# apache/cassandra

Hardware: AMD Instinct MI355X
Metric: compaction MB/s (input SSTable bytes merged+compressed) (higher is better)
Workload: dtype u8; 1 GPU; C2: 8x2GiB sstables, 10% key overlap, ~1KiB values, LZ4 16KiB chunks; sstables=8, overlap_pct=10, clustering_rows=0, tombstone_pct=0, range_tomb_pct=0, parallelism=token-independent shards x1, no collectives, storage=/tmp/gpuc_bench, input_uncompressed_bytes_per_rank=17182763435

## Files before the change

### cassandra_amd/csrc/gpucompact.cpp

```cpp
#include "kernels.hip"
#include "kernels_rows.hip"
#include "bti_core.h"
#include "sstable_meta.h"
#include "sstable_out.h"
#include "../../include/gpucompact.h"

#include <algorithm>
#include <cmath>
#include <cstdio>
#include <cstring>
#include <map>
#include <set>
#include <memory>
#include <mutex>
#include <stdexcept>
#include <string>
#include <thread>
#include <future>
#include <functional>
#include <atomic>
#include <fcntl.h>
#include <unistd.h>
#include <vector>

// ... 666 lines not shown
    m.has_partition_deletions = hst.has_partition_deletions != 0;
    memcpy(m.part_size_hist, hst.part_size_hist, sizeof(m.part_size_hist));
    memcpy(m.cells_hist, hst.cells_hist, sizeof(m.cells_hist));
}

struct OutputImage {
    uint64_t g0 = 0, g1 = 0;
    uint64_t total_unc = 0, total_idx = 0;
    uint32_t n_chunks = 0;
    const DevBuf *slots = nullptr, *csize = nullptr, *ccrc = nullptr;
    const DevBuf *out_index = nullptr, *bloom = nullptr;
    uint8_t* h_index = nullptr;
    uint64_t words = 0;
    HBloomSpec bs{};
    OutStats hst{};
    const std::vector<Event>* ev_c = nullptr;
    bool index_late = false;
};

static void drain_and_finish(const OutputImage& im, const OutPartsBuf& opb, const SerParams2& sp,
                             const DevBuf& d_tomb, uint32_t tomb_cap, const TableTypes& types,
                             const OutputOptions& opt, hipStream_t stream, hipStream_t cstream,
                             hipEvent_t ev2, hipEvent_t ev4, WriteDeviceOut& w) {
    const std::string& out_base = opt.base;
    const bool snappy_out = opt.snappy, bti_out = opt.bti;
    const int wslot = opt.wslot;
    const uint32_t OCL = opt.chunk_len;
    const uint32_t SLOT_STRIDE = snappy_out ? snp_slot_stride(OCL) : lz4_slot_stride(OCL);
    const uint32_t SLAB = (512u << 20) / OCL;
    const uint32_t n_chunks = im.n_chunks;
    const uint32_t n_slabs = n_chunks ? (n_chunks + SLAB - 1) / SLAB : 0;
    const uint64_t total_unc = im.total_unc, total_idx = im.total_idx, words = im.words;
    uint8_t* const h_index = im.h_index;
    const OutStats& hst = im.hst;
    const HBloomSpec& bs = im.bs;
    std::string data_path = out_base + "-Data.db";
    write_file(data_path, nullptr, 0);
    const uint64_t worst_slab = (uint64_t)SLAB * ((uint64_t)SLOT_STRIDE + 4);
    const int NSLOTS = 4;
    uint8_t* h_slab0 = (uint8_t*)g_pin_out[wslot][0].get(worst_slab * NSLOTS);
    if (!h_slab0) throw std::runtime_error("pinned out alloc failed");
    DevBuf d_gat[2], d_foff[2];
    if (n_slabs) {
        d_gat[0].alloc(worst_slab); d_gat[1].alloc(worst_slab);
        d_foff[0].alloc((uint64_t)SLAB * 8); d_foff[1].alloc((uint64_t)SLAB * 8);
    }
    std::vector<uint32_t> cs(n_chunks);
    std::vector<uint64_t> foff_h[2];
    foff_h[0].resize(SLAB); foff_h[1].resize(SLAB);
    std::future<void> wfut[NSLOTS];
    double t_drain0 = 0, t_drain1 = 0;
    {
        struct timespec tsd; clock_gettime(CLOCK_MONOTONIC, &tsd);
        t_drain0 = tsd.tv_sec * 1e3 + tsd.tv_nsec / 1e6;
    }
    uint64_t file_off = 0;
    double tw_comp = 0, tw_d2h = 0, tw_wfut = 0;
    auto wallm = []() {
        struct timespec t; clock_gettime(CLOCK_MONOTONIC, &t);
        return t.tv_sec * 1e3 + t.tv_nsec / 1e6;
    };
    for (uint32_t i = 0; i < n_slabs; i++) {
        uint32_t cb = i * SLAB, m = std::min(SLAB, n_chunks - cb);
        HIP_CHECK(hipStreamWaitEvent(cstream, (*im.ev_c)[i], 0));
        HIP_CHECK(hipMemcpyAsync(cs.data() + cb, im.csize->as<uint32_t>() + cb, (uint64_t)m * 4,
                                 hipMemcpyDeviceToHost, cstream));
        double tq0 = wallm();
        HIP_CHECK(hipStreamSynchronize(cstream));
        tw_comp += wallm() - tq0;
        auto& fo = foff_h[i & 1];
        uint64_t acc = 0;
        for (uint32_t j = 0; j < m; j++) { fo[j] = acc; acc += cs[cb + j]; }
        uint64_t slab_bytes = acc + (uint64_t)m * 4;
        HIP_CHECK(hipMemcpyAsync(d_foff[i & 1].p, fo.data(), (uint64_t)m * 8,
                                 hipMemcpyHostToDevice, cstream));
        hipLaunchKernelGGL(k_chunk_gather, dim3(m), dim3(WAVE), 0, cstream,
                           im.slots->as<uint8_t>() + (uint64_t)cb * SLOT_STRIDE,
                           im.csize->as<uint32_t>() + cb, im.ccrc->as<uint32_t>() + cb,
                           d_foff[i & 1].as<uint64_t>(), d_gat[i & 1].as<uint8_t>(), m,
                           SLOT_STRIDE);
        int slot = (int)(i % NSLOTS);
        double tq1 = wallm();
        if (wfut[slot].valid()) wfut[slot].get();
        tw_wfut += wallm() - tq1;
        uint8_t* hbuf = h_slab0 + (uint64_t)slot * worst_slab;
        HIP_CHECK(hipMemcpyAsync(hbuf, d_gat[i & 1].p, slab_bytes, hipMemcpyDeviceToHost, cstream));
        double tq2 = wallm();
        HIP_CHECK(hipStreamSynchronize(cstream));
        tw_d2h += wallm() - tq2;
        uint64_t off0 = file_off;
        wfut[slot] = std::async(std::launch::async, [=]() {
            pwrite_range(data_path, hbuf, slab_bytes, off0, 4);
        });
        file_off += slab_bytes;
    }
    {
        double tq3 = wallm();
        for (int sfin = 0; sfin < NSLOTS; sfin++)
            if (wfut[sfin].valid()) wfut[sfin].get();
        tw_wfut += wallm() - tq3;
    }
    if (g_trace)
        fprintf(stderr, "[drain] slabs=%u wait_compress=%.0fms wait_d2h=%.0fms wait_write=%.0fms\n",
                n_slabs, tw_comp, tw_d2h, tw_wfut);
    {
        struct timespec tsd; clock_gettime(CLOCK_MONOTONIC, &tsd);
        t_drain1 = tsd.tv_sec * 1e3 + tsd.tv_nsec / 1e6;
    }
    w.compressed_len = file_off;
    TR("wsd: drain done");
    if (im.index_late) {
        HIP_CHECK(hipStreamWaitEvent(cstream, ev2, 0));
        HIP_CHECK(hipMemcpyAsync(h_index, im.out_index->p, total_idx, hipMemcpyDeviceToHost, cstream));
        HIP_CHECK(hipStreamSynchronize(cstream));
    }
    HIP_CHECK(hipEventRecord(ev4, stream));

    {
        std::vector<uint8_t> h_bloom(words * 8);
        std::vector<uint32_t> h_crc(n_chunks);
        TR("wsd: tail vectors");
        HIP_CHECK(hipMemcpy(h_bloom.data(), im.bloom->p, words * 8, hipMemcpyDeviceToHost));
        TR("wsd: bloom d2h");
        if (n_chunks)
            HIP_CHECK(hipMemcpy(h_crc.data(), im.ccrc->p, (uint64_t)n_chunks * 4, hipMemcpyDeviceToHost));
        HIP_CHECK(hipStreamSynchronize(stream));
        HIP_CHECK(hipStreamSynchronize(cstream));
        TR("wsd: tail synced");
        std::future<uint32_t> fut_digest =
            std::async(std::launch::async, [&]() { return fold_digest(h_crc, cs); });
        std::future<bytes> fut_summary;
        if (!bti_out)
            fut_summary = std::async(std::launch::async,
                                     [&]() { return summary_db(h_index, total_idx); });

        std::vector<uint32_t> tombs;
        if (hst.tomb_count) {
            uint64_t nt = std::min<uint64_t>(hst.tomb_count, tomb_cap);
            tombs.resize(nt);
            HIP_CHECK(hipMemcpy(tombs.data(), d_tomb.p, nt * 4, hipMemcpyDeviceToHost));
            if (hst.tomb_count > tomb_cap)
                throw std::runtime_error("tombstone list overflow (internal cap)");
        }
        OutMeta m{};
        {
            const uint64_t n_groups = im.g1 - im.g0;
            DevBuf d_kh;
            d_kh.alloc(n_groups * 8 + 8);
            uint32_t blocks = (uint32_t)((n_groups + 255) / 256);
            if (n_groups)
                hipLaunchKernelGGL(k_key_hash2, dim3(blocks), dim3(256), 0, stream, opb.op,
                                   im.g1, d_kh.as<uint64_t>(), im.g0);
            std::vector<uint64_t> kh(n_groups);
            std::vector<uint8_t> keep(n_groups);
            if (n_groups) {
                HIP_CHECK(hipStreamSynchronize(stream));
                HIP_CHECK(hipMemcpy(kh.data(), d_kh.p, n_groups * 8, hipMemcpyDeviceToHost));
                HIP_CHECK(hipMemcpy(keep.data(), opb.op.keep + im.g0, n_groups, hipMemcpyDeviceToHost));
            }
            m.key_hashes.reserve(n_groups);
            for (uint64_t g2 = 0; g2 < n_groups; g2++)
                if (keep[g2]) m.key_hashes.push_back(kh[g2]);
        }
        fill_meta_from_stats(m, hst, sp.hs, types);
        for (uint32_t tv : tombs) m.tomb_hist[tv]++;
        m.compression_ratio = total_unc ? (double)(w.compressed_len - (uint64_t)n_chunks * 4) / (double)total_unc : -1.0;
        if (hst.partitions_out) {
            uint64_t fg = hst.first_group, lg = hst.last_group;
            for (int which = 0; which < 2; which++) {
                uint64_t g = which ? lg : fg;
                uint64_t ka;
                uint16_t kl;
                HIP_CHECK(hipMemcpy(&ka, opb.op.key_addr + g, 8, hipMemcpyDeviceToHost));
                HIP_CHECK(hipMemcpy(&kl, opb.op.klen + g, 2, hipMemcpyDeviceToHost));
                bytes kb(kl);
                HIP_CHECK(hipMemcpy(kb.data(), (const void*)ka, kl, hipMemcpyDeviceToHost));
                (which ? m.last_key : m.first_key) = kb;
            }
        }
        TR("wsd: meta built");
        uint32_t digest = fut_digest.get();

        TR("wsd: digest done");
        struct timespec ts0, ts1;
        clock_gettime(CLOCK_MONOTONIC, &ts0);
        if (bti_out) {
            bti::bytes parts_img, rows_img;
            std::vector<int32_t> ckw;
            for (auto& t : types.clustering_types) ckw.push_back(type_width(t));
            build_bti_from_index_image(h_index, total_idx, total_unc, ckw, &parts_img, &rows_img);
            write_file(out_base + "-Partitions.db", parts_img);
            write_file(out_base + "-Rows.db", rows_img);
        } else {
            write_file_parallel(out_base + "-Index.db", h_index, total_idx, 4);
        }
        write_file(out_base + "-Filter.db", filter_db(bs.k, h_bloom));
        write_file(out_base + "-CompressionInfo.db",
                   compression_info_db(snappy_out, OCL, total_unc, cs));
        write_file(out_base + "-Digest.crc32", digest_text(digest));
        write_file(out_base + "-Statistics.db", serialize_statistics_out(m));
        if (!bti_out) write_file(out_base + "-Summary.db", fut_summary.get());
        write_file(out_base + "-TOC.txt", toc_text(bti_out));
        clock_gettime(CLOCK_MONOTONIC, &ts1);
        TR("wsd: components written");
        w.ms_io = (ts1.tv_sec - ts0.tv_sec) * 1e3 + (ts1.tv_nsec - ts0.tv_nsec) / 1e6;
        w.ms_d2h = t_drain1 - t_drain0;
    }
}

static WriteDeviceOut write_sstable_device(const OutPartsBuf& opb, const UnfColsBuf& rows,
                                           uint64_t n_groups, SerParams2 sp, DevBuf& d_stats,
                                           DevBuf& d_tomb, uint32_t tomb_cap,
                                           const TableTypes& types, const OutputOptions& opt,
                                           hipStream_t stream) {
    WriteDeviceOut w;
    if (!chunk_len_supported(opt.chunk_len))
        throw unsupported_error("unsupported output chunk_length " + std::to_string(opt.chunk_len) +
                                CHUNK_LEN_WHY);
    const std::string& out_base = opt.base;
    const bool snappy_out = opt.snappy, bti_out = opt.bti;
    const int wslot = opt.wslot;
    const uint32_t OCL = opt.chunk_len;
// ... 48 lines not shown
    w.rows = hst.rows_out;
    w.cells = hst.total_cells;

    HBloomSpec bs = bloom_spec_001();
    uint64_t num_bits = w.partitions * (uint64_t)bs.buckets + 20;
    uint64_t words = num_bits ? ((num_bits - 1) >> 6) + 1 : 1;
    DevBuf d_out_data, d_out_index, d_bloom;
    d_out_data.alloc(total_unc);
    d_out_index.alloc(total_idx);
    d_bloom.alloc(words * 8);
    HIP_CHECK(hipMemsetAsync(d_bloom.p, 0, words * 8, stream));
    HIP_CHECK(hipEventRecord(ev1, stream));
    int NSEG = n_groups >= 4096 && total_unc > (256ull << 20) ? 8 : 1;
    if (const char* e = getenv("GPUC_NSEG")) NSEG = std::max(1, std::min(64, atoi(e)));
    if (n_groups < 4096) NSEG = 1;
    std::vector<uint64_t> seg_g(NSEG + 1), seg_end_byte(NSEG);
    if (NSEG > 1) {
        seg_g[0] = 0;
        seg_g[NSEG] = n_groups;
        for (int j = 1; j < NSEG; j++) seg_g[j] = n_groups * (uint64_t)j / NSEG;
        for (int j = 0; j < NSEG - 1; j++)
            HIP_CHECK(hipMemcpy(&seg_end_byte[j], d_psize.as<uint64_t>() + seg_g[j + 1], 8,
                                hipMemcpyDeviceToHost));
        seg_end_byte[NSEG - 1] = total_unc;
    } else {
        seg_g[0] = 0;
        seg_g[NSEG] = n_groups;
        seg_end_byte[NSEG - 1] = total_unc;
    }
    auto launch_serialize_seg = [&](int j) {
        uint32_t waves_per_block = 4;
        uint64_t gs = seg_g[j], ge = seg_g[j + 1];
        uint64_t blocks = (std::max<uint64_t>(ge - gs, 1) + waves_per_block - 1) / waves_per_block;
        if (ge > gs)
            hipLaunchKernelGGL(k_serialize_rows, dim3((uint32_t)blocks),
                               dim3(WAVE * waves_per_block), 0, stream, opb.op, rows.uc, ge,
                               sp, d_psize.as<uint64_t>(), d_isize.as<uint64_t>(),
                               d_nblocks.as<uint32_t>(), d_infsz.as<uint64_t>(),
                               d_out_data.as<uint8_t>(), d_out_index.as<uint8_t>(),
                               d_bloom.as<uint32_t>(), words * 64, bs.k, gs);
    };
    int seg_issued = 0;
    if (NSEG == 1) {
        launch_serialize_seg(0);
        seg_issued = 1;
        HIP_CHECK(hipEventRecord(ev2, stream));
    }

    if ((total_unc + OCL - 1) / OCL > 0xFFFFFFFFull)
        throw std::runtime_error("output too large for this chunk_length");
    uint32_t n_chunks = (uint32_t)((total_unc + OCL - 1) / OCL);
    const uint32_t SLAB = (512u << 20) / OCL;
    uint32_t n_slabs = n_chunks ? (n_chunks + SLAB - 1) / SLAB : 0;
    DevBuf d_slots, d_csize, d_ccrc;
    d_slots.alloc((uint64_t)n_chunks * SLOT_STRIDE + 16);
    d_csize.alloc((uint64_t)n_chunks * 4 + 16);
    d_ccrc.alloc((uint64_t)n_chunks * 4 + 16);
    uint8_t* h_index = (uint8_t*)g_pin_out[wslot][1].get(total_idx ? total_idx : 1);
    if (!h_index) throw std::runtime_error("pinned out alloc failed");
    if (NSEG == 1) {
        HIP_CHECK(hipStreamWaitEvent(cstream, ev2, 0));
        HIP_CHECK(hipMemcpyAsync(h_index, d_out_index.p, total_idx, hipMemcpyDeviceToHost, cstream));
    }

    std::vector<Event> ev_c(n_slabs);
    for (uint32_t i = 0; i < n_slabs; i++) {
        uint32_t cb = i * SLAB, m = std::min(SLAB, n_chunks - cb);
        if (NSEG > 1) {
            uint64_t slab_end = std::min<uint64_t>((uint64_t)(cb + m) * OCL, total_unc);
            while (seg_issued < NSEG && (seg_issued ? seg_end_byte[seg_issued - 1] : 0) < slab_end)
                launch_serialize_seg(seg_issued++);
            if (seg_issued == NSEG) {
                HIP_CHECK(hipEventRecord(ev2, stream));
                seg_issued++;
            }
        }
        launch_chunk_compress(snappy_out, d_out_data.as<uint8_t>() + (uint64_t)cb * OCL,
                              total_unc - (uint64_t)cb * OCL,
                              d_slots.as<uint8_t>() + (uint64_t)cb * SLOT_STRIDE,
                              d_csize.as<uint32_t>() + cb, d_ccrc.as<uint32_t>() + cb, m, OCL,
                              SLOT_STRIDE, stream);
        HIP_CHECK(hipEventRecord(ev_c[i], stream));
    }
    if (NSEG > 1 && seg_issued <= NSEG) {
        while (seg_issued < NSEG) launch_serialize_seg(seg_issued++);
        HIP_CHECK(hipEventRecord(ev2, stream));
    }
    HIP_CHECK(hipEventRecord(ev3, stream));
    TR("wsd: compress issued");

    OutputImage im;
    im.g0 = 0;
    im.g1 = n_groups;
    im.total_unc = total_unc;
    im.total_idx = total_idx;
    im.n_chunks = n_chunks;
    im.slots = &d_slots;
    im.csize = &d_csize;
    im.ccrc = &d_ccrc;
    im.out_index = &d_out_index;
    im.bloom = &d_bloom;
    im.h_index = h_index;
    im.words = words;
    im.bs = bs;
    im.hst = hst;
    im.ev_c = &ev_c;
    im.index_late = NSEG > 1;
    drain_and_finish(im, opb, sp, d_tomb, tomb_cap, types, opt, stream, cstream, ev2, ev4, w);
    w.uncompressed_len = total_unc;
    float t01, t12, t23;
    HIP_CHECK(hipEventElapsedTime(&t01, ev0, ev1));
    HIP_CHECK(hipEventElapsedTime(&t12, ev1, ev2));
    HIP_CHECK(hipEventElapsedTime(&t23, ev2, ev3));
    w.ms_sizes = t01;
    w.ms_serialize = t12;
    w.ms_compress = t23;
    return w;
}

static double size_split_margin() {
    if (const char* e = getenv("GPUC_SPLIT_MARGIN")) return std::max(0.0, atof(e));
    return 0.01;
}
// ... 208 lines not shown
        im.g0 = g0;
        im.g1 = g1;
        im.total_unc = P_h[g1] - B;
        im.n_chunks = (uint32_t)((im.total_unc + OCL - 1) / OCL);
        const uint32_t full = (uint32_t)(im.total_unc / OCL);
        if (full > cp.chunks_done || im.n_chunks > cp.cap_chunks)
            throw std::runtime_error("size split: chunk bookkeeping");
        if (im.n_chunks > full) {
            launch_chunk_compress(opt.snappy, d_out_data.as<uint8_t>() + B + (uint64_t)full * OCL,
                                  im.total_unc - (uint64_t)full * OCL,
                                  cp.slots.as<uint8_t>() + (uint64_t)full * SLOT_STRIDE,
                                  cp.csize.as<uint32_t>() + full, cp.ccrc.as<uint32_t>() + full, 1,
                                  OCL, SLOT_STRIDE, stream);
            cp.chunks_compressed++;
        }
        const uint32_t SLAB = (512u << 20) / OCL;
        std::vector<Event> ev_c((im.n_chunks + SLAB - 1) / SLAB);
        for (auto& e : ev_c) HIP_CHECK(hipEventRecord(e, stream));
        HIP_CHECK(hipMemcpyAsync(&im.total_idx, d_isize.as<uint64_t>() + g1, 8, hipMemcpyDeviceToHost, stream));
        init_outstats(d_stats_k, stream);
        {
            const uint32_t blocks = (uint32_t)((g1 - g0 + 255) / 256);
            hipLaunchKernelGGL(k_collect_rows, dim3(blocks), dim3(256), 0, stream, opb.op, rows.uc,
                               g1, sp.sch.n_cols, sp.sch.n_cpx, d_stats_k.as<OutStats>(),
                               d_tomb.as<uint32_t>(), tomb_cap, g0);
            hipLaunchKernelGGL(k_part_hists, dim3(blocks), dim3(256), 0, stream,
                               d_psize.as<uint64_t>(), d_cells.as<uint64_t>(), g1,
                               d_stats_k.as<OutStats>(), d_ps_off.as<int64_t>(),
                               (int32_t)ps_off_h.size(), d_ch_off.as<int64_t>(),
                               (int32_t)ch_off_h.size(), g0);
        }
        HIP_CHECK(hipStreamSynchronize(stream));
        HIP_CHECK(hipMemcpy(&im.hst, d_stats_k.p, sizeof(OutStats), hipMemcpyDeviceToHost));
        const uint64_t num_bits = im.hst.partitions_out * (uint64_t)bs.buckets + 20;
        im.words = ((num_bits - 1) >> 6) + 1;
        im.bs = bs;
        d_bloom.alloc(im.words * 8);
        HIP_CHECK(hipMemsetAsync(d_bloom.p, 0, im.words * 8, stream));
        hipLaunchKernelGGL(k_bloom_rows, dim3((uint32_t)((g1 - g0 + 255) / 256)), dim3(256), 0,
                           stream, opb.op, g1, d_bloom.as<uint32_t>(), im.words * 64, bs.k, g0);
        HIP_CHECK(hipEventRecord(ev2, stream));
        im.slots = &cp.slots;
        im.csize = &cp.csize;
        im.ccrc = &cp.ccrc;
        im.out_index = &d_out_index;
        im.bloom = &d_bloom;
        im.h_index = (uint8_t*)g_pin_out[opt.wslot][1].get(im.total_idx ? im.total_idx : 1);
        if (!im.h_index) throw std::runtime_error("pinned out alloc failed");
        im.ev_c = &ev_c;
        im.index_late = true;
        OutputOptions opt_k = opt;
        opt_k.base = output_base_plus(opt.base, tot.n_outputs);
        WriteDeviceOut w;
        drain_and_finish(im, opb, sp, d_tomb, tomb_cap, types, opt_k, stream, cstream, ev2, ev4, w);
        if (g_trace)
            fprintf(stderr, "[split] output %u groups=[%llu,%llu) unc=%llu comp=%llu windows=%u\n",
                    tot.n_outputs, (unsigned long long)g0, (unsigned long long)g1,
                    (unsigned long long)im.total_unc, (unsigned long long)w.compressed_len,
                    cp.windows);
        tot.n_outputs++;
        tot.partitions += im.hst.partitions_out;
        tot.rows += im.hst.rows_out;
        tot.cells += im.hst.total_cells;
        tot.uncompressed_len += im.total_unc;
        tot.compressed_len += w.compressed_len;
        tot.ms_d2h += w.ms_d2h;
        tot.ms_io += w.ms_io;
        chunks_written += im.n_chunks;
        windows_total += cp.windows;
// ... 1953 lines not shown
```

### cassandra_amd/csrc/sstable_out.h

```cpp
#pragma once
#include "codec.h"
#include "bti_core.h"
#include "sstable_meta.h"

#include <algorithm>
#include <cmath>
#include <cstdio>
#include <cstring>
#include <map>
#include <set>
#include <stdexcept>
#include <string>
#include <thread>
#include <fcntl.h>
#include <unistd.h>
#include <vector>

namespace gpuc {

inline void put_be16(bytes& o, uint16_t v) { o.push_back(v >> 8); o.push_back((uint8_t)v); }
inline void put_be32(bytes& o, uint32_t v) { for (int i = 3; i >= 0; i--) o.push_back((uint8_t)(v >> (8 * i))); }
inline void put_be64(bytes& o, uint64_t v) { for (int i = 7; i >= 0; i--) o.push_back((uint8_t)(v >> (8 * i))); }
inline void put_uvint(bytes& o, uint64_t v) {
    uint8_t tmp[9];
// ... 110 lines not shown
    int64_t hdr_min_ts, hdr_min_ldt;
    int32_t hdr_min_ttl;
    TableTypes types;
    int64_t min_timestamp, max_timestamp, min_ldt, max_ldt;
    int32_t min_ttl, max_ttl;
    uint64_t total_rows, total_cells;
    bool has_partition_deletions;
    bytes first_key, last_key;
    std::map<uint32_t, uint32_t> tomb_hist;
    double compression_ratio;
    uint64_t part_size_hist[156];
    uint64_t cells_hist[119];
    std::vector<uint64_t> key_hashes;
};

inline bytes serialize_statistics_out(const OutMeta& m) {
    bytes validation;
    {
        std::string pn = "org.apache.cassandra.dht.Murmur3Partitioner";
        put_be16(validation, (uint16_t)pn.size());
        validation.insert(validation.end(), pn.begin(), pn.end());
        uint64_t fp;
        double fpv = 0.01;
        memcpy(&fp, &fpv, 8);
        put_be64(validation, fp);
    }
    bytes compaction = hll_bytes(m.key_hashes);
    const std::vector<std::string>& ck_types = m.types.clustering_types;
    bytes stats;
    {
        static const std::vector<int64_t> ps_off = est_hist_offsets(155);
        static const std::vector<int64_t> ch_off = est_hist_offsets(118);
        put_est_hist(stats, ps_off, m.part_size_hist);
        put_est_hist(stats, ch_off, m.cells_hist);
        put_be64(stats, (uint64_t)-1LL); put_be32(stats, 0);
        put_be64(stats, (uint64_t)m.min_timestamp);
        put_be64(stats, (uint64_t)m.max_timestamp);
        put_be32(stats, ldt_u32(m.min_ldt));
        put_be32(stats, ldt_u32(m.max_ldt));
        put_be32(stats, (uint32_t)m.min_ttl);
        put_be32(stats, (uint32_t)m.max_ttl);
        uint64_t cr; double crv = m.compression_ratio; memcpy(&cr, &crv, 8); put_be64(stats, cr);
// ... 62 lines not shown
        put_be32(out, crc32_update_bitwise(0, comps[i]->data(), comps[i]->size()));
    }
    return out;
}

struct HBloomSpec { int k; int buckets; };
inline HBloomSpec bloom_spec_001() { return {5, 10}; }

inline bytes filter_db(int hash_count, const std::vector<uint8_t>& bloom_words) {
    bytes f;
    put_be32(f, (uint32_t)hash_count);
    put_be32(f, (uint32_t)(bloom_words.size() / 8));
    f.insert(f.end(), bloom_words.begin(), bloom_words.end());
    return f;
}

inline bytes compression_info_db(bool snappy, uint32_t chunk_len, uint64_t total_unc,
                                 const std::vector<uint32_t>& chunk_sizes) {
    bytes ci;
    std::string algo = snappy ? "SnappyCompressor" : "LZ4Compressor";
    put_be16(ci, (uint16_t)algo.size());
    ci.insert(ci.end(), algo.begin(), algo.end());
    put_be32(ci, 0);
    put_be32(ci, chunk_len);
    put_be32(ci, 0x7FFFFFFF);
    put_be64(ci, total_unc);
    put_be32(ci, (uint32_t)chunk_sizes.size());
    uint64_t acc = 0;
    for (size_t i = 0; i < chunk_sizes.size(); i++) { put_be64(ci, acc + (uint64_t)i * 4); acc += chunk_sizes[i]; }
    return ci;
// ... 19 lines not shown
                                 (uint8_t)(chunk_crcs[c] >> 8), (uint8_t)chunk_crcs[c]};
                d = comb.combine(d, crc32_update_bitwise(0, cb, 4), 4);
                l += chunk_sizes[c] + 4;
            }
            pcrc[t] = d;
            plen[t] = l;
        });
    }
    for (auto& x : th) x.join();
    uint32_t dg = 0;
    for (int t = 0; t < nth; t++) dg = comb.combine(dg, pcrc[t], plen[t]);
    return dg;
}
inline std::string digest_text(uint32_t digest) { return std::to_string(digest); }

inline std::string toc_text(bool bti) {
    return bti ? "Data.db\nStatistics.db\nDigest.crc32\nTOC.txt\nCompressionInfo.db\nFilter.db\nPartitions.db\nRows.db\n"
               : "Data.db\nStatistics.db\nDigest.crc32\nTOC.txt\nCompressionInfo.db\nFilter.db\nIndex.db\nSummary.db\n";
}

inline bytes summary_db(const uint8_t* idx, uint64_t idx_len) {
    const uint32_t MIN_INTERVAL = 128;
    bytes entries, s;
    std::vector<uint32_t> offs;
    const uint8_t *first_k = nullptr, *last_k = nullptr;
    uint32_t first_kl = 0, last_kl = 0;
    uint64_t q = 0, part_i = 0;
    while (q < idx_len) {
        uint64_t entry_off = q;
        uint32_t klen = ((uint32_t)idx[q] << 8) | idx[q + 1];
// ... 17 lines not shown
    put_be32(s, 128);
    put_be32(s, cnt);
    for (uint32_t o : offs) {
        uint32_t v = o + 4 * cnt;
        for (int b = 0; b < 4; b++) s.push_back((uint8_t)(v >> (8 * b)));
    }
    s.insert(s.end(), entries.begin(), entries.end());
    if (first_k) {
        put_be32(s, first_kl);
        s.insert(s.end(), first_k, first_k + first_kl);
        put_be32(s, last_kl);
        s.insert(s.end(), last_k, last_k + last_kl);
    }
    return s;
}

inline void build_bti_from_index_image(const uint8_t* idx, uint64_t idx_len, uint64_t data_total,
                                       const std::vector<int32_t>& ck_w,
                                       bti::bytes* partitions_out, bti::bytes* rows_out) {
    uint64_t p = 0;
    bytes rows_file;
    std::vector<bti::BtiKeyEntry> pes;
    std::vector<bti::BtiRowIndexBlockSpec> pending_specs;
    std::vector<size_t> pending_idx;
    std::vector<uint64_t> part_positions;
    auto uvint = [&]() -> uint64_t { return uvint_get(idx, &p); };
    auto be_n = [&](int n) -> uint64_t {
        uint64_t v = 0;
        for (int i = 0; i < n; i++) v = (v << 8) | idx[p++];
        return v;
// ... 131 lines not shown
```

Measured before the change: 8118 MB/s.

## Overlap SSTable tail metadata work with data drain via background workers

Moves the post-drain tail work (index D2H, Summary, Filter, CompressionInfo, digest fold, key-hash HLL and tombstone histogram) off the critical path. Index pieces are copied and written incrementally by a worker thread during the slab drain, metadata is computed by a separate worker after async copies into pinned arenas, and CompressionInfo and the digest are folded per slab with a sliced CRC combiner. This aims to shorten the serial tail after Data.db is written, at the cost of extra threads, more pinned memory and added synchronisation complexity.

Measured after the change: 7732 MB/s. 4.8% lower.

```diff
diff --git a/cassandra_amd/csrc/gpucompact.cpp b/cassandra_amd/csrc/gpucompact.cpp
--- a/cassandra_amd/csrc/gpucompact.cpp
+++ b/cassandra_amd/csrc/gpucompact.cpp
@@ -7,6 +7,7 @@
 
 #include <algorithm>
 #include <cmath>
+#include <condition_variable>
 #include <cstdio>
 #include <cstring>
 #include <map>
@@ -704,12 +705,223 @@
     uint64_t words = 0;
     HBloomSpec bs{};
     OutStats hst{};
+    uint32_t slab = 0;
     const std::vector<Event>* ev_c = nullptr;
-    bool index_late = false;
+    struct IndexPiece {
+        hipEvent_t ev;
+        uint64_t end;
+        uint32_t before_slab;
+    };
+    std::vector<IndexPiece> pieces;
+    static constexpr uint32_t NO_SLAB = 0xFFFFFFFFu;
+    uint32_t ev2_before_slab = NO_SLAB;
 };
 
-static void drain_and_finish(const OutputImage& im, const OutPartsBuf& opb, const SerParams2& sp,
-                             const DevBuf& d_tomb, uint32_t tomb_cap, const TableTypes& types,
+static uint32_t slab_chunks(uint32_t chunk_len) {
+    uint64_t mb = 512;
+    if (const char* e = getenv("GPUC_SLAB_MB")) mb = (uint64_t)std::max(1, std::min(512, atoi(e)));
+    return (uint32_t)std::max<uint64_t>(1, (mb << 20) / chunk_len);
+}
+
+struct TailWorker {
+    std::thread th;
+    std::exception_ptr err;
+    TailWorker() = default;
+    TailWorker(const TailWorker&) = delete;
+    TailWorker& operator=(const TailWorker&) = delete;
+    template <class F> void start(int device, F fn) {
+        th = std::thread([this, device, fn]() {
+            try {
+                HIP_CHECK(hipSetDevice(device));
+                fn();
+            } catch (...) {
+                err = std::current_exception();
+            }
+        });
+    }
+    void join() {
+        if (th.joinable()) th.join();
+        if (err) {
+            std::exception_ptr e = err;
+            err = nullptr;
+            std::rethrow_exception(e);
+        }
+    }
+    ~TailWorker() {
+        if (th.joinable()) th.join();
+    }
+};
+
+struct EarlyMeta {
+    DevBuf d_kh;
+    Event ev_ready, ev_done;
+    const uint64_t* h_kh = nullptr;
+    const uint32_t* h_tombs = nullptr;
+    const uint8_t* h_keep = nullptr;
+    uint64_t n_groups = 0, n_tombs = 0;
+    OutMeta m{};
+    bytes hll;
+    TailWorker worker;
+
+    void issue(const OutPartsBuf& opb, uint64_t g0, uint64_t g1, const OutStats& hst,
+               const HeaderStats& hs, const TableTypes& types, const DevBuf& d_tomb,
+               uint32_t tomb_cap, int wslot, hipStream_t stream, hipStream_t copy_stream) {
+        if (hst.tomb_count > tomb_cap)
+            throw std::runtime_error("tombstone list overflow (internal cap)");
+        n_groups = g1 - g0;
+        n_tombs = hst.tomb_count;
+        fill_meta_from_stats(m, hst, hs, types);
+        if (hst.partitions_out) {
+            for (int which = 0; which < 2; which++) {
+                uint64_t g = which ? hst.last_group : hst.first_group;
+                uint64_t ka;
+                uint16_t kl;
+                HIP_CHECK(hipMemcpy(&ka, opb.op.key_addr + g, 8, hipMemcpyDeviceToHost));
+                HIP_CHECK(hipMemcpy(&kl, opb.op.klen + g, 2, hipMemcpyDeviceToHost));
+                bytes kb(kl);
+                HIP_CHECK(hipMemcpy(kb.data(), (const void*)ka, kl, hipMemcpyDeviceToHost));
+                (which ? m.last_key : m.first_key) = kb;
+            }
+        }
+        d_kh.alloc(n_groups * 8 + 8);
+        if (n_groups)
+            hipLaunchKernelGGL(k_key_hash2, dim3((uint32_t)((n_groups + 255) / 256)), dim3(256), 0,
+                               stream, opb.op, g1, d_kh.as<uint64_t>(), g0);
+        uint8_t* arena = (uint8_t*)g_pin_out[wslot][2].get(n_groups * 9 + n_tombs * 4 + 64);
+        if (!arena) throw std::runtime_error("pinned out alloc failed");
+        h_kh = (const uint64_t*)arena;
+        h_tombs = (const uint32_t*)(arena + n_groups * 8);
+        h_keep = arena + n_groups * 8 + n_tombs * 4;
+        if (copy_stream != stream) {
+            HIP_CHECK(hipEventRecord(ev_ready, stream));
+            HIP_CHECK(hipStreamWaitEvent(copy_stream, ev_ready, 0));
+        }
+        if (n_groups) {
+            HIP_CHECK(hipMemcpyAsync((void*)h_kh, d_kh.p, n_groups * 8, hipMemcpyDeviceToHost, copy_stream));
+            HIP_CHECK(hipMemcpyAsync((void*)h_keep, opb.op.keep + g0, n_groups, hipMemcpyDeviceToHost, copy_stream));
+        }
+        if (n_tombs)
+            HIP_CHECK(hipMemcpyAsync((void*)h_tombs, d_tomb.p, n_tombs * 4, hipMemcpyDeviceToHost, copy_stream));
+        HIP_CHECK(hipEventRecord(ev_done, copy_stream));
+        int device = 0;
+        HIP_CHECK(hipGetDevice(&device));
+        worker.start(device, [this]() {
+            HIP_CHECK(hipEventSynchronize(ev_done));
+            double t0 = trace_wall();
+            m.key_hashes.reserve(n_groups);
+            for (uint64_t g = 0; g < n_groups; g++)
+                if (h_keep[g]) m.key_hashes.push_back(h_kh[g]);
+            double t1 = trace_wall();
+            hll = hll_bytes(m.key_hashes);
+            for (uint64_t i = 0; i < n_tombs; i++) m.tomb_hist[h_tombs[i]]++;
+            if (g_trace)
+                fprintf(stderr, "[meta worker] filter %.1f ms, hll + tombstones %.1f ms\n", t1 - t0,
+                        trace_wall() - t1);
+        });
+    }
+};
+
+struct IndexJob {
+    std::string base;
+    bool bti = false;
+    const uint8_t* h_index = nullptr;
+    uint64_t total_idx = 0, total_unc = 0;
+    const uint8_t* h_bloom = nullptr;
+    uint64_t words = 0;
+    int bloom_k = 0;
+    std::vector<int32_t> ck_widths;
+    Event ev_all;
+
+    std::mutex mu;
+    std::condition_variable cv;
+    uint64_t avail = 0;
+    bool all_enqueued = false, abort = false;
+    TailWorker worker;
+
+    void publish(uint64_t bytes_on_host) {
+        {
+            std::lock_guard<std::mutex> g(mu);
+            if (bytes_on_host <= avail) return;
+            avail = bytes_on_host;
+        }
+        cv.notify_one();
+    }
+    void publish_all_enqueued() {
+        {
+            std::lock_guard<std::mutex> g(mu);
+            all_enqueued = true;
+        }
+        cv.notify_one();
+    }
+    ~IndexJob() {
+        {
+            std::lock_guard<std::mutex> g(mu);
+            abort = true;
+        }
+        cv.notify_one();
+    }
+    void start(int device) {
+        worker.start(device, [this]() { run(); });
+    }
+    void run() {
+        int fd = -1;
+        struct Closer {
+            int& fd;
+            ~Closer() { if (fd >= 0) close(fd); }
+        } closer{fd};
+        const std::string index_path = base + "-Index.db";
+        if (!bti) {
+            fd = open(index_path.c_str(), O_WRONLY | O_CREAT | O_TRUNC, 0666);
+            if (fd < 0) throw std::runtime_error("cannot create " + index_path);
+        }
+        SummaryBuilder sb;
+        uint64_t done = 0;
+        double busy = 0;
+        auto take = [&](uint64_t upto) {
+            if (bti || upto <= done) return;
+            double t0 = trace_wall();
+            sb.add(h_index, done, upto);
+            while (done < upto) {
+                ssize_t wr = pwrite(fd, h_index + done, upto - done, (off_t)done);
+                if (wr <= 0) throw std::runtime_error("short write " + index_path);
+                done += (uint64_t)wr;
+            }
+            busy += trace_wall() - t0;
+        };
+        for (;;) {
+            uint64_t upto;
+            bool last;
+            {
+                std::unique_lock<std::mutex> g(mu);
+                cv.wait(g, [&]() { return abort || all_enqueued || avail > done; });
+                if (abort) return;
+                upto = avail;
+                last = all_enqueued;
+            }
+            if (last) break;
+            take(upto);
+        }
+        HIP_CHECK(hipEventSynchronize(ev_all));
+        const double t0 = trace_wall(), busy_early = busy;
+        take(total_idx);
+        if (bti) {
+            bti::bytes parts_img, rows_img;
+            build_bti_from_index_image(h_index, total_idx, total_unc, ck_widths, &parts_img, &rows_img);
+            write_file(base + "-Partitions.db", parts_img);
+            write_file(base + "-Rows.db", rows_img);
+        } else {
+            close(fd);
+            fd = -1;
+            write_file(base + "-Summary.db", sb.finish());
+        }
+        write_filter_db(base + "-Filter.db", bloom_k, h_bloom, words);
+        if (g_trace)
+            fprintf(stderr, "[index worker] pieces before the end %.1f ms, after it %.1f ms\n",
+                    busy_early, trace_wall() - t0);
+    }
+};
+
+static void drain_and_finish(const OutputImage& im, EarlyMeta& meta, const TableTypes& types,
                              const OutputOptions& opt, hipStream_t stream, hipStream_t cstream,
                              hipEvent_t ev2, hipEvent_t ev4, WriteDeviceOut& w) {
     const std::string& out_base = opt.base;
@@ -717,27 +929,69 @@
     const int wslot = opt.wslot;
     const uint32_t OCL = opt.chunk_len;
     const uint32_t SLOT_STRIDE = snappy_out ? snp_slot_stride(OCL) : lz4_slot_stride(OCL);
-    const uint32_t SLAB = (512u << 20) / OCL;
+    const uint32_t SLAB = im.slab;
     const uint32_t n_chunks = im.n_chunks;
     const uint32_t n_slabs = n_chunks ? (n_chunks + SLAB - 1) / SLAB : 0;
     const uint64_t total_unc = im.total_unc, total_idx = im.total_idx, words = im.words;
     uint8_t* const h_index = im.h_index;
-    const OutStats& hst = im.hst;
-    const HBloomSpec& bs = im.bs;
+    int device = 0;
+    HIP_CHECK(hipGetDevice(&device));
     std::string data_path = out_base + "-Data.db";
     write_file(data_path, nullptr, 0);
     const uint64_t worst_slab = (uint64_t)SLAB * ((uint64_t)SLOT_STRIDE + 4);
     const int NSLOTS = 4;
     uint8_t* h_slab0 = (uint8_t*)g_pin_out[wslot][0].get(worst_slab * NSLOTS);
     if (!h_slab0) throw std::runtime_error("pinned out alloc failed");
+    uint8_t* h_tail = (uint8_t*)g_pin_out[wslot][3].get(words * 8 + (uint64_t)n_chunks * 8 + 64);
+    if (!h_tail) throw std::runtime_error("pinned out alloc failed");
+    uint8_t* const h_bloom = h_tail;
+    uint32_t* const cs = (uint32_t*)(h_tail + words * 8);
+    uint32_t* const h_crc = cs + n_chunks;
     DevBuf d_gat[2], d_foff[2];
     if (n_slabs) {
         d_gat[0].alloc(worst_slab); d_gat[1].alloc(worst_slab);
         d_foff[0].alloc((uint64_t)SLAB * 8); d_foff[1].alloc((uint64_t)SLAB * 8);
     }
-    std::vector<uint32_t> cs(n_chunks);
     std::vector<uint64_t> foff_h[2];
     foff_h[0].resize(SLAB); foff_h[1].resize(SLAB);
+    CompressionInfoBuilder cinfo(snappy_out, OCL, total_unc, n_chunks);
+    DigestFold digest;
+
+    IndexJob ij;
+    ij.base = out_base;
+    ij.bti = bti_out;
+    ij.h_index = h_index;
+    ij.total_idx = total_idx;
+    ij.total_unc = total_unc;
+    ij.h_bloom = h_bloom;
+    ij.words = words;
+    ij.bloom_k = im.bs.k;
+    if (bti_out)
+        for (auto& t : types.clustering_types) ij.ck_widths.push_back(type_width(t));
+    ij.start(device);
+    size_t piece_next = 0;
+    uint64_t idx_enq = 0;
+    bool idx_all = false;
+    auto enqueue_index = [&](uint32_t slab_i) {
+        if (idx_all) return;
+        for (; piece_next < im.pieces.size() && im.pieces[piece_next].before_slab <= slab_i; piece_next++) {
+            const OutputImage::IndexPiece& pc = im.pieces[piece_next];
+            if (pc.end <= idx_enq) continue;
+            HIP_CHECK(hipStreamWaitEvent(cstream, pc.ev, 0));
+            HIP_CHECK(hipMemcpyAsync(h_index + idx_enq, im.out_index->as<uint8_t>() + idx_enq,
+                                     pc.end - idx_enq, hipMemcpyDeviceToHost, cstream));
+            idx_enq = pc.end;
+        }
+        if (im.ev2_before_slab > slab_i) return;
+        HIP_CHECK(hipStreamWaitEvent(cstream, ev2, 0));
+        if (total_idx > idx_enq)
+            HIP_CHECK(hipMemcpyAsync(h_index + idx_enq, im.out_index->as<uint8_t>() + idx_enq,
+                                     total_idx - idx_enq, hipMemcpyDeviceToHost, cstream));
+        HIP_CHECK(hipMemcpyAsync(h_bloom, im.bloom->p, words * 8, hipMemcpyDeviceToHost, cstream));
+        HIP_CHECK(hipEventRecord(ij.ev_all, cstream));
+        idx_all = true;
+        ij.publish_all_enqueued();
+    };
     std::future<void> wfut[NSLOTS];
     double t_drain0 = 0, t_drain1 = 0;
     {
@@ -745,19 +999,24 @@
         t_drain0 = tsd.tv_sec * 1e3 + tsd.tv_nsec / 1e6;
     }
     uint64_t file_off = 0;
-    double tw_comp = 0, tw_d2h = 0, tw_wfut = 0;
+    double tw_comp = 0, tw_d2h = 0, tw_wfut = 0, tw_fold = 0;
     auto wallm = []() {
         struct timespec t; clock_gettime(CLOCK_MONOTONIC, &t);
         return t.tv_sec * 1e3 + t.tv_nsec / 1e6;
     };
     for (uint32_t i = 0; i < n_slabs; i++) {
         uint32_t cb = i * SLAB, m = std::min(SLAB, n_chunks - cb);
+        enqueue_index(i);
+        const uint64_t idx_ahead = idx_enq;
         HIP_CHECK(hipStreamWaitEvent(cstream, (*im.ev_c)[i], 0));
-        HIP_CHECK(hipMemcpyAsync(cs.data() + cb, im.csize->as<uint32_t>() + cb, (uint64_t)m * 4,
+        HIP_CHECK(hipMemcpyAsync(cs + cb, im.csize->as<uint32_t>() + cb, (uint64_t)m * 4,
+                                 hipMemcpyDeviceToHost, cstream));
+        HIP_CHECK(hipMemcpyAsync(h_crc + cb, im.ccrc->as<uint32_t>() + cb, (uint64_t)m * 4,
                                  hipMemcpyDeviceToHost, cstream));
         double tq0 = wallm();
         HIP_CHECK(hipStreamSynchronize(cstream));
         tw_comp += wallm() - tq0;
+        ij.publish(idx_ahead);
         auto& fo = foff_h[i & 1];
         uint64_t acc = 0;
         for (uint32_t j = 0; j < m; j++) { fo[j] = acc; acc += cs[cb + j]; }
@@ -775,6 +1034,10 @@
         tw_wfut += wallm() - tq1;
         uint8_t* hbuf = h_slab0 + (uint64_t)slot * worst_slab;
         HIP_CHECK(hipMemcpyAsync(hbuf, d_gat[i & 1].p, slab_bytes, hipMemcpyDeviceToHost, cstream));
+        double tq4 = wallm();
+        cinfo.add(cs + cb, m);
+        digest.add(h_crc + cb, cs + cb, m);
+        tw_fold += wallm() - tq4;
         double tq2 = wallm();
         HIP_CHECK(hipStreamSynchronize(cstream));
         tw_d2h += wallm() - tq2;
@@ -791,111 +1054,36 @@
         tw_wfut += wallm() - tq3;
     }
     if (g_trace)
-        fprintf(stderr, "[drain] slabs=%u wait_compress=%.0fms wait_d2h=%.0fms wait_write=%.0fms\n",
-                n_slabs, tw_comp, tw_d2h, tw_wfut);
+        fprintf(stderr,
+                "[drain] slabs=%u wait_compress=%.0fms wait_d2h=%.0fms wait_write=%.0fms fold=%.0fms\n",
+                n_slabs, tw_comp, tw_d2h, tw_wfut, tw_fold);
     {
         struct timespec tsd; clock_gettime(CLOCK_MONOTONIC, &tsd);
         t_drain1 = tsd.tv_sec * 1e3 + tsd.tv_nsec / 1e6;
     }
     w.compressed_len = file_off;
     TR("wsd: drain done");
-    if (im.index_late) {
-        HIP_CHECK(hipStreamWaitEvent(cstream, ev2, 0));
-        HIP_CHECK(hipMemcpyAsync(h_index, im.out_index->p, total_idx, hipMemcpyDeviceToHost, cstream));
-        HIP_CHECK(hipStreamSynchronize(cstream));
-    }
+    enqueue_index(OutputImage::NO_SLAB);
     HIP_CHECK(hipEventRecord(ev4, stream));
 
-    {
-        std::vector<uint8_t> h_bloom(words * 8);
-        std::vector<uint32_t> h_crc(n_chunks);
-        TR("wsd: tail vectors");
-        HIP_CHECK(hipMemcpy(h_bloom.data(), im.bloom->p, words * 8, hipMemcpyDeviceToHost));
-        TR("wsd: bloom d2h");
-        if (n_chunks)
-            HIP_CHECK(hipMemcpy(h_crc.data(), im.ccrc->p, (uint64_t)n_chunks * 4, hipMemcpyDeviceToHost));
-        HIP_CHECK(hipStreamSynchronize(stream));
-        HIP_CHECK(hipStreamSynchronize(cstream));
-        TR("wsd: tail synced");
-        std::future<uint32_t> fut_digest =
-            std::async(std::launch::async, [&]() { return fold_digest(h_crc, cs); });
-        std::future<bytes> fut_summary;
-        if (!bti_out)
-            fut_summary = std::async(std::launch::async,
-                                     [&]() { return summary_db(h_index, total_idx); });
-
-        std::vector<uint32_t> tombs;
-        if (hst.tomb_count) {
-            uint64_t nt = std::min<uint64_t>(hst.tomb_count, tomb_cap);
-            tombs.resize(nt);
-            HIP_CHECK(hipMemcpy(tombs.data(), d_tomb.p, nt * 4, hipMemcpyDeviceToHost));
-            if (hst.tomb_count > tomb_cap)
-                throw std::runtime_error("tombstone list overflow (internal cap)");
-        }
-        OutMeta m{};
-        {
-            const uint64_t n_groups = im.g1 - im.g0;
-            DevBuf d_kh;
-            d_kh.alloc(n_groups * 8 + 8);
-            uint32_t blocks = (uint32_t)((n_groups + 255) / 256);
-            if (n_groups)
-                hipLaunchKernelGGL(k_key_hash2, dim3(blocks), dim3(256), 0, stream, opb.op,
-                                   im.g1, d_kh.as<uint64_t>(), im.g0);
-            std::vector<uint64_t> kh(n_groups);
-            std::vector<uint8_t> keep(n_groups);
-            if (n_groups) {
-                HIP_CHECK(hipStreamSynchronize(stream));
-                HIP_CHECK(hipMemcpy(kh.data(), d_kh.p, n_groups * 8, hipMemcpyDeviceToHost));
-                HIP_CHECK(hipMemcpy(keep.data(), opb.op.keep + im.g0, n_groups, hipMemcpyDeviceToHost));
-            }
-            m.key_hashes.reserve(n_groups);
-            for (uint64_t g2 = 0; g2 < n_groups; g2++)
-                if (keep[g2]) m.key_hashes.push_back(kh[g2]);
-        }
-        fill_meta_from_stats(m, hst, sp.hs, types);
-        for (uint32_t tv : tombs) m.tomb_hist[tv]++;
-        m.compression_ratio = total_unc ? (double)(w.compressed_len - (uint64_t)n_chunks * 4) / (double)total_unc : -1.0;
-        if (hst.partitions_out) {
-            uint64_t fg = hst.first_group, lg = hst.last_group;
-            for (int which = 0; which < 2; which++) {
-                uint64_t g = which ? lg : fg;
-                uint64_t ka;
-                uint16_t kl;
-                HIP_CHECK(hipMemcpy(&ka, opb.op.key_addr + g, 8, hipMemcpyDeviceToHost));
-                HIP_CHECK(hipMemcpy(&kl, opb.op.klen + g, 2, hipMemcpyDeviceToHost));
-                bytes kb(kl);
-                HIP_CHECK(hipMemcpy(kb.data(), (const void*)ka, kl, hipMemcpyDeviceToHost));
-                (which ? m.last_key : m.first_key) = kb;
-            }
-        }
-        TR("wsd: meta built");
-        uint32_t digest = fut_digest.get();
-
-        TR("wsd: digest done");
-        struct timespec ts0, ts1;
-        clock_gettime(CLOCK_MONOTONIC, &ts0);
-        if (bti_out) {
-            bti::bytes parts_img, rows_img;
-            std::vector<int32_t> ckw;
-            for (auto& t : types.clustering_types) ckw.push_back(type_width(t));
-            build_bti_from_index_image(h_index, total_idx, total_unc, ckw, &parts_img, &rows_img);
-            write_file(out_base + "-Partitions.db", parts_img);
-            write_file(out_base + "-Rows.db", rows_img);
-        } else {
-            write_file_parallel(out_base + "-Index.db", h_index, total_idx, 4);
-        }
-        write_file(out_base + "-Filter.db", filter_db(bs.k, h_bloom));
-        write_file(out_base + "-CompressionInfo.db",
-                   compression_info_db(snappy_out, OCL, total_unc, cs));
-        write_file(out_base + "-Digest.crc32", digest_text(digest));
-        write_file(out_base + "-Statistics.db", serialize_statistics_out(m));
-        if (!bti_out) write_file(out_base + "-Summary.db", fut_summary.get());
-        write_file(out_base + "-TOC.txt", toc_text(bti_out));
-        clock_gettime(CLOCK_MONOTONIC, &ts1);
-        TR("wsd: components written");
-        w.ms_io = (ts1.tv_sec - ts0.tv_sec) * 1e3 + (ts1.tv_nsec - ts0.tv_nsec) / 1e6;
-        w.ms_d2h = t_drain1 - t_drain0;
-    }
+    meta.worker.join();
+    TR("wsd: meta joined");
+    OutMeta& m = meta.m;
+    m.compression_ratio = total_unc ? (double)(w.compressed_len - (uint64_t)n_chunks * 4) / (double)total_unc : -1.0;
+    struct timespec ts0, ts1;
+    clock_gettime(CLOCK_MONOTONIC, &ts0);
+    write_file(out_base + "-CompressionInfo.db", cinfo.finish());
+    write_file(out_base + "-Digest.crc32", digest_text(digest.digest()));
+    write_file(out_base + "-Statistics.db", serialize_statistics_out(m, &meta.hll));
+    TR("wsd: small components written");
+    ij.worker.join();
+    HIP_CHECK(hipStreamSynchronize(stream));
+    HIP_CHECK(hipStreamSynchronize(cstream));
+    write_file(out_base + "-TOC.txt", toc_text(bti_out));
+    clock_gettime(CLOCK_MONOTONIC, &ts1);
+    TR("wsd: components written");
+    w.ms_io = (ts1.tv_sec - ts0.tv_sec) * 1e3 + (ts1.tv_nsec - ts0.tv_nsec) / 1e6;
+    w.ms_d2h = t_drain1 - t_drain0;
 }
 
 static WriteDeviceOut write_sstable_device(const OutPartsBuf& opb, const UnfColsBuf& rows,
@@ -974,14 +1162,18 @@
     int NSEG = n_groups >= 4096 && total_unc > (256ull << 20) ? 8 : 1;
     if (const char* e = getenv("GPUC_NSEG")) NSEG = std::max(1, std::min(64, atoi(e)));
     if (n_groups < 4096) NSEG = 1;
-    std::vector<uint64_t> seg_g(NSEG + 1), seg_end_byte(NSEG);
+    std::vector<uint64_t> seg_g(NSEG + 1), seg_end_byte(NSEG), seg_end_idx(NSEG);
+    seg_end_idx[NSEG - 1] = total_idx;
     if (NSEG > 1) {
         seg_g[0] = 0;
         seg_g[NSEG] = n_groups;
         for (int j = 1; j < NSEG; j++) seg_g[j] = n_groups * (uint64_t)j / NSEG;
-        for (int j = 0; j < NSEG - 1; j++)
+        for (int j = 0; j < NSEG - 1; j++) {
             HIP_CHECK(hipMemcpy(&seg_end_byte[j], d_psize.as<uint64_t>() + seg_g[j + 1], 8,
                                 hipMemcpyDeviceToHost));
+            HIP_CHECK(hipMemcpy(&seg_end_idx[j], d_isize.as<uint64_t>() + seg_g[j + 1], 8,
+                                hipMemcpyDeviceToHost));
+        }
         seg_end_byte[NSEG - 1] = total_unc;
     } else {
         seg_g[0] = 0;
@@ -1000,17 +1192,31 @@
                                d_out_data.as<uint8_t>(), d_out_index.as<uint8_t>(),
                                d_bloom.as<uint32_t>(), words * 64, bs.k, gs);
     };
+    EarlyMeta meta;
+    meta.issue(opb, 0, n_groups, hst, sp.hs, types, d_tomb, tomb_cap, wslot, stream,
+               getenv("GPUC_META_ON_MAIN") ? stream : (hipStream_t)cstream);
+    TR("wsd: early meta issued");
+    std::vector<Event> ev_seg(NSEG - 1);
+    OutputImage im;
+    auto launch_segment = [&](int j, uint32_t before_slab) {
+        launch_serialize_seg(j);
+        if (j < NSEG - 1) {
+            HIP_CHECK(hipEventRecord(ev_seg[j], stream));
+            im.pieces.push_back({ev_seg[j], seg_end_idx[j], before_slab});
+        }
+    };
     int seg_issued = 0;
     if (NSEG == 1) {
         launch_serialize_seg(0);
         seg_issued = 1;
         HIP_CHECK(hipEventRecord(ev2, stream));
+        im.ev2_before_slab = 0;
     }
 
     if ((total_unc + OCL - 1) / OCL > 0xFFFFFFFFull)
         throw std::runtime_error("output too large for this chunk_length");
     uint32_t n_chunks = (uint32_t)((total_unc + OCL - 1) / OCL);
-    const uint32_t SLAB = (512u << 20) / OCL;
+    const uint32_t SLAB = slab_chunks(OCL);
     uint32_t n_slabs = n_chunks ? (n_chunks + SLAB - 1) / SLAB : 0;
     DevBuf d_slots, d_csize, d_ccrc;
     d_slots.alloc((uint64_t)n_chunks * SLOT_STRIDE + 16);
@@ -1018,20 +1224,19 @@
     d_ccrc.alloc((uint64_t)n_chunks * 4 + 16);
     uint8_t* h_index = (uint8_t*)g_pin_out[wslot][1].get(total_idx ? total_idx : 1);
     if (!h_index) throw std::runtime_error("pinned out alloc failed");
-    if (NSEG == 1) {
-        HIP_CHECK(hipStreamWaitEvent(cstream, ev2, 0));
-        HIP_CHECK(hipMemcpyAsync(h_index, d_out_index.p, total_idx, hipMemcpyDeviceToHost, cstream));
-    }
 
     std::vector<Event> ev_c(n_slabs);
     for (uint32_t i = 0; i < n_slabs; i++) {
         uint32_t cb = i * SLAB, m = std::min(SLAB, n_chunks - cb);
         if (NSEG > 1) {
             uint64_t slab_end = std::min<uint64_t>((uint64_t)(cb + m) * OCL, total_unc);
-            while (seg_issued < NSEG && (seg_issued ? seg_end_byte[seg_issued - 1] : 0) < slab_end)
-                launch_serialize_seg(seg_issued++);
+            while (seg_issued < NSEG && (seg_issued ? seg_end_byte[seg_issued - 1] : 0) < slab_end) {
+                launch_segment(seg_issued, i);
+                seg_issued++;
+            }
             if (seg_issued == NSEG) {
                 HIP_CHECK(hipEventRecord(ev2, stream));
+                im.ev2_before_slab = i;
                 seg_issued++;
             }
         }
@@ -1043,13 +1248,12 @@
         HIP_CHECK(hipEventRecord(ev_c[i], stream));
     }
     if (NSEG > 1 && seg_issued <= NSEG) {
-        while (seg_issued < NSEG) launch_serialize_seg(seg_issued++);
+        for (; seg_issued < NSEG; seg_issued++) launch_segment(seg_issued, OutputImage::NO_SLAB);
         HIP_CHECK(hipEventRecord(ev2, stream));
     }
     HIP_CHECK(hipEventRecord(ev3, stream));
     TR("wsd: compress issued");
 
-    OutputImage im;
     im.g0 = 0;
     im.g1 = n_groups;
     im.total_unc = total_unc;
@@ -1064,9 +1268,9 @@
     im.words = words;
     im.bs = bs;
     im.hst = hst;
+    im.slab = SLAB;
     im.ev_c = &ev_c;
-    im.index_late = NSEG > 1;
-    drain_and_finish(im, opb, sp, d_tomb, tomb_cap, types, opt, stream, cstream, ev2, ev4, w);
+    drain_and_finish(im, meta, types, opt, stream, cstream, ev2, ev4, w);
     w.uncompressed_len = total_unc;
     float t01, t12, t23;
     HIP_CHECK(hipEventElapsedTime(&t01, ev0, ev1));
@@ -1305,7 +1509,8 @@
                                   OCL, SLOT_STRIDE, stream);
             cp.chunks_compressed++;
         }
-        const uint32_t SLAB = (512u << 20) / OCL;
+        const uint32_t SLAB = slab_chunks(OCL);
+        im.slab = SLAB;
         std::vector<Event> ev_c((im.n_chunks + SLAB - 1) / SLAB);
         for (auto& e : ev_c) HIP_CHECK(hipEventRecord(e, stream));
         HIP_CHECK(hipMemcpyAsync(&im.total_idx, d_isize.as<uint64_t>() + g1, 8, hipMemcpyDeviceToHost, stream));
@@ -1323,6 +1528,8 @@
         }
         HIP_CHECK(hipStreamSynchronize(stream));
         HIP_CHECK(hipMemcpy(&im.hst, d_stats_k.p, sizeof(OutStats), hipMemcpyDeviceToHost));
+        EarlyMeta meta;
+        meta.issue(opb, g0, g1, im.hst, sp.hs, types, d_tomb, tomb_cap, opt.wslot, stream, stream);
         const uint64_t num_bits = im.hst.partitions_out * (uint64_t)bs.buckets + 20;
         im.words = ((num_bits - 1) >> 6) + 1;
         im.bs = bs;
@@ -1339,11 +1546,11 @@
         im.h_index = (uint8_t*)g_pin_out[opt.wslot][1].get(im.total_idx ? im.total_idx : 1);
         if (!im.h_index) throw std::runtime_error("pinned out alloc failed");
         im.ev_c = &ev_c;
-        im.index_late = true;
+        im.ev2_before_slab = OutputImage::NO_SLAB;
         OutputOptions opt_k = opt;
         opt_k.base = output_base_plus(opt.base, tot.n_outputs);
         WriteDeviceOut w;
-        drain_and_finish(im, opb, sp, d_tomb, tomb_cap, types, opt_k, stream, cstream, ev2, ev4, w);
+        drain_and_finish(im, meta, types, opt_k, stream, cstream, ev2, ev4, w);
         if (g_trace)
             fprintf(stderr, "[split] output %u groups=[%llu,%llu) unc=%llu comp=%llu windows=%u\n",
                     tot.n_outputs, (unsigned long long)g0, (unsigned long long)g1,
diff --git a/cassandra_amd/csrc/sstable_out.h b/cassandra_amd/csrc/sstable_out.h
--- a/cassandra_amd/csrc/sstable_out.h
+++ b/cassandra_amd/csrc/sstable_out.h
@@ -148,7 +148,7 @@
     std::vector<uint64_t> key_hashes;
 };
 
-inline bytes serialize_statistics_out(const OutMeta& m) {
+inline bytes serialize_statistics_out(const OutMeta& m, const bytes* hll = nullptr) {
     bytes validation;
     {
         std::string pn = "org.apache.cassandra.dht.Murmur3Partitioner";
@@ -159,7 +159,7 @@
         memcpy(&fp, &fpv, 8);
         put_be64(validation, fp);
     }
-    bytes compaction = hll_bytes(m.key_hashes);
+    bytes compaction = hll ? *hll : hll_bytes(m.key_hashes);
     const std::vector<std::string>& ck_types = m.types.clustering_types;
     bytes stats;
     {
@@ -252,6 +252,18 @@
     f.insert(f.end(), bloom_words.begin(), bloom_words.end());
     return f;
 }
+inline void write_filter_db(const std::string& path, int hash_count, const uint8_t* bloom_words,
+                            uint64_t n_words) {
+    bytes head;
+    put_be32(head, (uint32_t)hash_count);
+    put_be32(head, (uint32_t)n_words);
+    FILE* f = fopen(path.c_str(), "wb");
+    if (!f) throw std::runtime_error("cannot create " + path);
+    bool ok = fwrite(head.data(), 1, head.size(), f) == head.size() &&
+              (n_words == 0 || fwrite(bloom_words, 1, n_words * 8, f) == n_words * 8);
+    if (fclose(f) != 0) ok = false;
+    if (!ok) throw std::runtime_error("short write " + path);
+}
 
 inline bytes compression_info_db(bool snappy, uint32_t chunk_len, uint64_t total_unc,
                                  const std::vector<uint32_t>& chunk_sizes) {
@@ -301,6 +313,91 @@
 }
 inline std::string digest_text(uint32_t digest) { return std::to_string(digest); }
 
+struct CompressionInfoBuilder {
+    bytes ci;
+    uint32_t n_chunks, added = 0;
+    uint64_t acc = 0;
+    CompressionInfoBuilder(bool snappy, uint32_t chunk_len, uint64_t total_unc, uint32_t n_chunks_)
+        : n_chunks(n_chunks_) {
+        std::string algo = snappy ? "SnappyCompressor" : "LZ4Compressor";
+        ci.reserve(2 + algo.size() + 24 + (size_t)n_chunks * 8);
+        put_be16(ci, (uint16_t)algo.size());
+        ci.insert(ci.end(), algo.begin(), algo.end());
+        put_be32(ci, 0);
+        put_be32(ci, chunk_len);
+        put_be32(ci, 0x7FFFFFFF);
+        put_be64(ci, total_unc);
+        put_be32(ci, n_chunks);
+    }
+    void add(const uint32_t* chunk_sizes, size_t n) {
+        if (n > (size_t)(n_chunks - added)) throw std::runtime_error("CompressionInfo: too many chunks");
+        for (size_t i = 0; i < n; i++) {
+            put_be64(ci, acc + (uint64_t)added * 4);
+            acc += chunk_sizes[i];
+            added++;
+        }
+    }
+    uint64_t data_len() const { return acc + (uint64_t)added * 4; }
+    const bytes& finish() const {
+        if (added != n_chunks) throw std::runtime_error("CompressionInfo: chunks missing");
+        return ci;
+    }
+};
+
+struct Crc32CombinerSliced {
+    std::vector<uint32_t> t;
+    uint32_t byte_tab[256];
+    Crc32CombinerSliced() : t((size_t)64 * 4 * 256) {
+        const Crc32Combiner c;
+        for (int k = 0; k < 64; k++)
+            for (int b = 0; b < 4; b++)
+                for (uint32_t v = 0; v < 256; v++)
+                    t[((size_t)k * 4 + b) * 256 + v] = gf2_times(c.pow[k], v << (8 * b));
+        for (uint32_t v = 0; v < 256; v++) {
+            uint32_t r = v;
+            for (int i = 0; i < 8; i++) r = (r & 1) ? 0xEDB88320u ^ (r >> 1) : r >> 1;
+            byte_tab[v] = r;
+        }
+    }
+    uint32_t combine(uint32_t crc1, uint32_t crc2, uint64_t len2) const {
+        if (len2 == 0) return crc1;
+        uint32_t c = crc1;
+        for (int k = 0; len2; len2 >>= 1, k++) {
+            if (!(len2 & 1)) continue;
+            const uint32_t* p = &t[(size_t)k * 1024];
+            c = p[c & 0xFF] ^ p[256 + ((c >> 8) & 0xFF)] ^ p[512 + ((c >> 16) & 0xFF)] ^ p[768 + (c >> 24)];
+        }
+        return c ^ crc2;
+    }
+    uint32_t extend_be32(uint32_t crc, uint32_t v) const {
+        crc = ~crc;
+        for (int s = 24; s >= 0; s -= 8) crc = byte_tab[(crc ^ (v >> s)) & 0xFF] ^ (crc >> 8);
+        return ~crc;
+    }
+};
+
+struct DigestFold {
+    uint32_t crc = 0;
+    uint64_t len = 0;
+    static const Crc32CombinerSliced& combiner() {
+        static const Crc32CombinerSliced comb;
+        return comb;
+    }
+    void add(const uint32_t* chunk_crcs, const uint32_t* chunk_sizes, size_t n) {
+        const Crc32CombinerSliced& comb = combiner();
+        for (size_t c = 0; c < n; c++) {
+            crc = comb.combine(crc, chunk_crcs[c], chunk_sizes[c]);
+            crc = comb.extend_be32(crc, chunk_crcs[c]);
+            len += (uint64_t)chunk_sizes[c] + 4;
+        }
+    }
+    void append(const DigestFold& next) {
+        crc = combiner().combine(crc, next.crc, next.len);
+        len += next.len;
+    }
+    uint32_t digest() const { return crc; }
+};
+
 inline std::string toc_text(bool bti) {
     return bti ? "Data.db\nStatistics.db\nDigest.crc32\nTOC.txt\nCompressionInfo.db\nFilter.db\nPartitions.db\nRows.db\n"
                : "Data.db\nStatistics.db\nDigest.crc32\nTOC.txt\nCompressionInfo.db\nFilter.db\nIndex.db\nSummary.db\n";
@@ -348,6 +445,58 @@
     }
     return s;
 }
+
+struct SummaryBuilder {
+    static constexpr uint32_t MIN_INTERVAL = 128;
+    bytes entries, first_key, last_key;
+    std::vector<uint32_t> offs;
+    uint64_t part_i = 0, walked = 0;
+    void add(const uint8_t* idx, uint64_t from, uint64_t to) {
+        if (from != walked) throw std::runtime_error("Summary: index pieces out of order");
+        uint64_t q = from;
+        const uint8_t* kp = nullptr;
+        uint32_t klen = 0;
+        while (q < to) {
+            uint64_t entry_off = q;
+            klen = ((uint32_t)idx[q] << 8) | idx[q + 1];
+            kp = idx + q + 2;
+            q += 2 + klen;
+            if (part_i == 0) first_key.assign(kp, kp + klen);
+            if (part_i % MIN_INTERVAL == 0) {
+                offs.push_back((uint32_t)entries.size());
+                entries.insert(entries.end(), kp, kp + klen);
+                for (int b = 0; b < 8; b++) entries.push_back((uint8_t)(entry_off >> (8 * b)));
+            }
+            (void)uvint_get(idx, &q);
+            q += uvint_get(idx, &q);
+            part_i++;
+        }
+        if (q != to) throw std::runtime_error("Summary: index piece ends inside an entry");
+        if (kp) last_key.assign(kp, kp + klen);
+        walked = to;
+    }
+    bytes finish() const {
+        bytes s;
+        uint32_t cnt = (uint32_t)offs.size();
+        put_be32(s, MIN_INTERVAL);
+        put_be32(s, cnt);
+        put_be64(s, 4ull * cnt + entries.size());
+        put_be32(s, 128);
+        put_be32(s, cnt);
+        for (uint32_t o : offs) {
+            uint32_t v = o + 4 * cnt;
+            for (int b = 0; b < 4; b++) s.push_back((uint8_t)(v >> (8 * b)));
+        }
+        s.insert(s.end(), entries.begin(), entries.end());
+        if (part_i) {
+            put_be32(s, (uint32_t)first_key.size());
+            s.insert(s.end(), first_key.begin(), first_key.end());
+            put_be32(s, (uint32_t)last_key.size());
+            s.insert(s.end(), last_key.begin(), last_key.end());
+        }
+        return s;
+    }
+};
 
 inline void build_bti_from_index_image(const uint8_t* idx, uint64_t idx_len, uint64_t data_total,
                                        const std::vector<int32_t>& ck_w,
```
